# denix56/SI-Mamba

Measured on AMD Instinct MI355X. Metric: point-clouds/sec (fwd+bwd), higher is better.
Workload: dtype f32; 1 GPU; PointMamba classifier train step (FPS+kNN grouping, encoder, spectral SAST ordering, 12 Mamba blocks d=384 at L=1024, head, AdamW), 1024 pts -> 128 patches; global_batch=64, per_gpu_batch=64, npoints=1024, patches=128, mamba_seq_len=1024, parallelism=dp1, communicator_ranks=1, library_gemm=tuned solution table (si_mamba_amd/tuned/gemm_gfx950.csv)

## Files before the change

include/simamba.h:

```cpp
#ifndef SIMAMBA_H_
#define SIMAMBA_H_

#include <stddef.h>

#ifdef __cplusplus
extern "C" {
#endif

#define SIMAMBA_ABI_VERSION 9

#define SIMAMBA_F32  0
#define SIMAMBA_BF16 1

#define SIMAMBA_OK            0
#define SIMAMBA_E_NULLPTR    -1
#define SIMAMBA_E_SHAPE      -2
#define SIMAMBA_E_DTYPE      -3
#define SIMAMBA_E_DSTATE     -4
#define SIMAMBA_E_WIDTH      -5
#define SIMAMBA_E_WORKSPACE  -6
#define SIMAMBA_E_GROUPS     -7
#define SIMAMBA_E_ALIGN      -8
#define SIMAMBA_E_VARIANT    -9

#define SIMAMBA_SCAN_CHUNK 128

#define SIMAMBA_SCAN_CKPT_ROW 128
#define SIMAMBA_SCAN_CKPT_SEQ 16

int         simamba_abi_version(void);
const char* simamba_strerror(int rc);
int         simamba_scan_num_chunks(int seqlen);
int         simamba_scan_fwd_auto_variant(int batch, int dim);
int         simamba_scan_ckpt_step(int batch, int dim, int seqlen, int dstate, int io_dtype);
long long   simamba_scan_ckpt_floats(int batch, int dim, int seqlen, int dstate, int ckpt_step);

#define SIMAMBA_SCAN_AUTO    0
#define SIMAMBA_SCAN_ROWSCAN 1
#define SIMAMBA_SCAN_LPC2    2
#define SIMAMBA_SCAN_LPC4    4
#define SIMAMBA_SCAN_MIX     6
int simamba_selective_scan_fwd(const void* u, const void* delta, const float* A,
                               const void* B, const void* C, const float* D, const void* z,
                               const float* delta_bias, void* out, float* x_ckpt,
                               float* last_state, int batch, int dim, int seqlen, int dstate,
                               int io_dtype, int delta_softplus, long long z_bstride,
                               long long bc_bstride, long long bc_nstride, long long bc_tstride,
                               int ckpt_step, int variant, void* stream);

int simamba_selective_scan_bwd(const void* u, const void* delta, const float* A,
                               const void* B, const void* C, const float* D, const void* z,
                               const float* delta_bias, const void* dout, const float* x_ckpt,
                               void* du, void* ddelta, float* dA, float* dB, float* dC,
                               float* dD, void* dz, float* ddelta_bias,
                               int batch, int dim, int seqlen, int dstate,
                               int io_dtype, int delta_softplus, long long z_bstride,
                               long long dz_bstride, long long bc_bstride, long long bc_nstride,
                               long long bc_tstride, int ckpt_step, void* stream);

int simamba_selective_scan_dt_fwd(const void* u, const void* xdbl, const void* wdt, const float* A, const float* D,
                                  const void* z, const float* delta_bias, void* out, float* x_ckpt, float* last_state,
                                  int batch, int dim, int seqlen, int dstate, int dt_rank, int io_dtype,
                                  long long z_bstride, long long xdbl_bstride, long long xdbl_tstride, int ckpt_step,
                                  int variant, void* stream);
int simamba_selective_scan_dt_bwd(const void* u, const void* xdbl, const void* wdt, const float* A, const float* D,
                                  const void* z, const float* delta_bias, const void* dout, const float* x_ckpt,
                                  void* du, void* ddelta, float* dA, float* dB, float* dC, float* dD, void* dz,
                                  float* ddelta_bias, int batch, int dim, int seqlen, int dstate, int dt_rank,
                                  int io_dtype, long long z_bstride, long long dz_bstride, long long xdbl_bstride,
                                  long long xdbl_tstride, void* stream);

int simamba_xdt_proj_fwd(const void* x, const void* wx, const void* wdt, void* xdbl, void* delta,
                         int batch, int D, int seqlen, int S, int R, int io_dtype, long long x_bstride,
                         void* stream);
int simamba_conv_xdt_proj_fwd(const void* x, const float* cw, const float* cb, const void* wx, const void* wdt,
                              void* xconv, void* xdbl, void* delta, int batch, int D, int seqlen, int S, int R,
                              int io_dtype, long long x_bstride, void* stream);

int simamba_seq_gather_fwd(const void* in, const int* idx, void* out, int batch, int channels, int G, int L,
                           long long out_bstride, int io_dtype, void* stream);
int simamba_seq_gather_bwd(const void* dout, const int* inv, void* din, int batch, int channels, int G, int L,
                           int R, long long dout_bstride, int io_dtype, void* stream);

int simamba_causal_conv1d_fwd(const void* x, const float* w, const float* bias, void* out,
                              int batch, int dim, int seqlen, int width, int silu,
                              int io_dtype, long long x_bstride, void* stream);
int simamba_causal_conv1d_bwd(const void* x, const float* w, const float* bias,
                              const void* dout, void* dx, float* dw, float* dbias,
                              int batch, int dim, int seqlen, int width, int silu,
                              int io_dtype, long long x_bstride, long long dx_bstride, void* stream);

int simamba_add_layer_norm_grid(int batch, int rows_per_batch);
int simamba_add_layer_norm_fwd(const void* hidden, const float* residual, const float* rowscale,
                               const float* weight, const float* bias, float* residual_out,
                               void* normed, float* mean, float* rstd, int batch, int rows_per_batch,
                               int dim, float eps, int hidden_dtype, int out_dtype, void* stream);
int simamba_add_layer_norm_bwd(const void* dnormed, const float* dresidual_out,
                               const float* residual_out, const float* mean, const float* rstd,
                               const float* weight, const float* rowscale, float* dresidual,
                               void* dhidden, float* dwb_partial, int batch, int rows_per_batch,
                               int dim, int hidden_dtype, int out_dtype, void* stream);

int simamba_out_proj_add_ln_fwd(const void* y, const void* w, const float* residual, const float* rowscale,
                                const float* gamma, const float* beta, float* residual_out, void* normed, float* mean,
                                float* rstd, int batch, int K, int L, int C, float eps, int out_dtype, void* stream);

int simamba_in_proj_fwd(const void* x, const void* w, void* xz, int batch, int L, int C, int M, int io_dtype,
                        void* stream);

int simamba_bn_relu_grid(long long rows);
int simamba_bn_relu_fwd(const void* x, const float* gterm, int group, const float* weight, const float* bias,
                        float* running_mean, float* running_var, float momentum, float eps, int training,
                        void* y, float* mean, float* invstd, float* partial, long long rows, int C,
                        long long ld, int io_dtype, void* stream);
int simamba_bn_relu_bwd(const void* dy, const void* x, const float* gterm, int group, const float* weight,
                        const float* bias, const float* mean, const float* invstd, void* dx, float* dgterm,
                        int dgroup, float* dweight, float* dbias, float* partial, long long rows, int C,
                        long long ld, int io_dtype, int training, void* stream);
int simamba_group_max_fwd(const void* x, void* out, unsigned char* idx, long long groups, int n, int C,
                          int io_dtype, void* stream);
int simamba_group_max_bwd(const void* dout, const unsigned char* idx, void* dx, long long groups, int n, int C,
                          int io_dtype, void* stream);

int simamba_three_nn(const float* xyz1, const float* xyz2, int* idx, float* weight, int batch, int N, int S,
                     void* stream);
int simamba_three_interpolate_fwd(const void* feats, const int* idx, const float* weight, void* out, int batch,
                                  int N, int S, int C, int io_dtype, void* stream);
int simamba_three_interpolate_bwd(const void* dout, const int* idx, const float* weight, float* dfeats, int batch,
                                  int N, int S, int C, int io_dtype, void* stream);

int simamba_chamfer_fwd(const float* pred, const float* gt, float* dist, unsigned char* idx1, unsigned char* idx2,
                        long long pairs, int n, int m, void* stream);
int simamba_chamfer_bwd(const float* pred, const float* gt, const float* ddist, const unsigned char* idx1,
                        const unsigned char* idx2, float* dpred, long long pairs, int n, int m, void* stream);

int simamba_knn_group(const float* points, const float* centers, long long* idx, int batch, int N, int G, int K,
                      void* stream);

#define SIMAMBA_SPEC_SYMMETRIC   0x01u
#define SIMAMBA_SPEC_SELF_LOOP   0x02u
#define SIMAMBA_SPEC_BINARY      0x04u
#define SIMAMBA_SPEC_MATRIX_SYM  0x08u
#define SIMAMBA_SPEC_SMALLEST    0x10u
#define SIMAMBA_SPEC_SIGMA_MEAN  0x20u

int simamba_knn_graph(const float* points, float* adj, void* workspace, size_t ws_bytes,
                      int B, int G, int F, int knn, float alpha, unsigned flags, void* stream);

int simamba_laplacian_topk(const float* adj, float* evals, float* evecs, long long* order,
                           float* all_evals, float* all_evecs, int B, int G, int k,
                           unsigned flags, void* stream);

size_t simamba_spectral_workspace_bytes(int B, int G);

int simamba_spectral_topk(const float* centers, float* evals, float* evecs, long long* order,
                          void* workspace, size_t ws_bytes, int B, int G, int knn, float alpha,
                          int k, unsigned flags, void* stream);

int simamba_farthest_point_sample(const float* points, long long* idx, float* centers, int B, int N,
                                  int K, void* stream);

int simamba_argsort_rows(const float* vals, long long* idx, int rows, int n, void* stream);

#ifdef __cplusplus
}
#endif
#endif
```

si_mamba_amd/_lib.py:

```python
from __future__ import annotations

import ctypes
import os
from ctypes import c_char_p, c_float, c_int, c_longlong, c_size_t, c_uint, c_void_p

_HERE = os.path.dirname(os.path.abspath(__file__))
LIB_PATH = os.path.join(_HERE, "libsimamba_hip.so")

F32, BF16 = 0, 1

SPEC_SYMMETRIC = 0x01
SPEC_SELF_LOOP = 0x02
SPEC_BINARY = 0x04
SPEC_MATRIX_SYM = 0x08
SPEC_SMALLEST = 0x10
SPEC_SIGMA_MEAN = 0x20

SCAN_AUTO, SCAN_ROWSCAN, SCAN_LPC2, SCAN_LPC4, SCAN_MIX = 0, 1, 2, 4, 6
CKPT_ROW, CKPT_SEQ = 128, 16

_P = c_void_p
_LL = c_longlong
ABI_VERSION = 9
SIGNATURES = {
    "simamba_abi_version": (c_int, []),
    "simamba_strerror": (c_char_p, [c_int]),
    "simamba_scan_num_chunks": (c_int, [c_int]),
    "simamba_scan_fwd_auto_variant": (c_int, [c_int, c_int]),
    "simamba_scan_ckpt_step": (c_int, [c_int, c_int, c_int, c_int, c_int]),
    "simamba_scan_ckpt_floats": (_LL, [c_int, c_int, c_int, c_int, c_int]),
    "simamba_selective_scan_fwd": (c_int, [_P, _P, _P, _P, _P, _P, _P, _P, _P, _P, _P,
                                           c_int, c_int, c_int, c_int, c_int, c_int,
                                           _LL, _LL, _LL, _LL, c_int, c_int, _P]),
    "simamba_selective_scan_bwd": (c_int, [_P, _P, _P, _P, _P, _P, _P, _P, _P, _P,
                                           _P, _P, _P, _P, _P, _P, _P, _P,
                                           c_int, c_int, c_int, c_int, c_int, c_int,
                                           _LL, _LL, _LL, _LL, _LL, c_int, _P]),
    "simamba_selective_scan_dt_fwd": (c_int, [_P, _P, _P, _P, _P, _P, _P, _P, _P, _P,
                                              c_int, c_int, c_int, c_int, c_int, c_int,
                                              _LL, _LL, _LL, c_int, c_int, _P]),
    "simamba_selective_scan_dt_bwd": (c_int, [_P, _P, _P, _P, _P, _P, _P, _P, _P,
                                              _P, _P, _P, _P, _P, _P, _P, _P,
                                              c_int, c_int, c_int, c_int, c_int, c_int,
                                              _LL, _LL, _LL, _LL, _P]),
    "simamba_xdt_proj_fwd": (c_int, [_P, _P, _P, _P, _P, c_int, c_int, c_int, c_int, c_int, c_int, _LL, _P]),
    "simamba_conv_xdt_proj_fwd": (c_int, [_P, _P, _P, _P, _P, _P, _P, _P, c_int, c_int, c_int, c_int, c_int, c_int, _LL,
                                          _P]),
    "simamba_seq_gather_fwd": (c_int, [_P, _P, _P, c_int, c_int, c_int, c_int, _LL, c_int, _P]),
    "simamba_seq_gather_bwd": (c_int, [_P, _P, _P, c_int, c_int, c_int, c_int, c_int, _LL, c_int, _P]),
    "simamba_causal_conv1d_fwd": (c_int, [_P, _P, _P, _P, c_int, c_int, c_int, c_int, c_int, c_int, _LL, _P]),
    "simamba_causal_conv1d_bwd": (c_int, [_P, _P, _P, _P, _P, _P, _P,
                                          c_int, c_int, c_int, c_int, c_int, c_int, _LL, _LL, _P]),
    "simamba_add_layer_norm_grid": (c_int, [c_int, c_int]),
    "simamba_add_layer_norm_fwd": (c_int, [_P, _P, _P, _P, _P, _P, _P, _P, _P, c_int, c_int, c_int, c_float,
                                           c_int, c_int, _P]),
    "simamba_add_layer_norm_bwd": (c_int, [_P, _P, _P, _P, _P, _P, _P, _P, _P, _P, c_int, c_int, c_int,
                                           c_int, c_int, _P]),
    "simamba_out_proj_add_ln_fwd": (c_int, [_P, _P, _P, _P, _P, _P, _P, _P, _P, _P, c_int, c_int, c_int, c_int, c_float,
                                            c_int, _P]),
    "simamba_in_proj_fwd": (c_int, [_P, _P, _P, c_int, c_int, c_int, c_int, c_int, _P]),
    "simamba_bn_relu_grid": (c_int, [_LL]),
    "simamba_bn_relu_fwd": (c_int, [_P, _P, c_int, _P, _P, _P, _P, c_float, c_float, c_int, _P, _P, _P, _P, _LL, c_int,
                                    _LL, c_int, _P]),
    "simamba_bn_relu_bwd": (c_int, [_P, _P, _P, c_int, _P, _P, _P, _P, _P, _P, c_int, _P, _P, _P, _LL, c_int, _LL,
                                    c_int, c_int, _P]),
    "simamba_group_max_fwd": (c_int, [_P, _P, _P, _LL, c_int, c_int, c_int, _P]),
    "simamba_group_max_bwd": (c_int, [_P, _P, _P, _LL, c_int, c_int, c_int, _P]),
    "simamba_three_nn": (c_int, [_P, _P, _P, _P, c_int, c_int, c_int, _P]),
    "simamba_three_interpolate_fwd": (c_int, [_P, _P, _P, _P, c_int, c_int, c_int, c_int, c_int, _P]),
    "simamba_three_interpolate_bwd": (c_int, [_P, _P, _P, _P, c_int, c_int, c_int, c_int, c_int, _P]),
    "simamba_chamfer_fwd": (c_int, [_P, _P, _P, _P, _P, _LL, c_int, c_int, _P]),
    "simamba_chamfer_bwd": (c_int, [_P, _P, _P, _P, _P, _P, _LL, c_int, c_int, _P]),
    "simamba_knn_group": (c_int, [_P, _P, _P, c_int, c_int, c_int, c_int, _P]),
    "simamba_knn_graph": (c_int, [_P, _P, _P, c_size_t, c_int, c_int, c_int, c_int, c_float, c_uint, _P]),
    "simamba_laplacian_topk": (c_int, [_P, _P, _P, _P, _P, _P, c_int, c_int, c_int, c_uint, _P]),
    "simamba_spectral_workspace_bytes": (c_size_t, [c_int, c_int]),
    "simamba_spectral_topk": (c_int, [_P, _P, _P, _P, _P, c_size_t, c_int, c_int, c_int, c_float,
                                      c_int, c_uint, _P]),
    "simamba_argsort_rows": (c_int, [_P, _P, c_int, c_int, _P]),
    "simamba_farthest_point_sample": (c_int, [_P, _P, _P, c_int, c_int, c_int, _P]),
}

_lib = None


def load():
    global _lib
    if _lib is not None:
        return _lib
    if not os.path.exists(LIB_PATH):
        raise RuntimeError(
            f"{LIB_PATH} not found: build it with `python -c 'import __graft_entry__ as g; g.build()'` "
            "or `make -C si_mamba_amd/csrc`.  si_mamba_amd has no CPU / eager fallback.")
    lib = ctypes.CDLL(LIB_PATH)
    for name, (res, args) in SIGNATURES.items():
        fn = getattr(lib, name)
        fn.restype = res
        fn.argtypes = args
    got = lib.simamba_abi_version()
    if got != ABI_VERSION:
        raise RuntimeError(f"libsimamba_hip.so ABI version {got}, binding expects {ABI_VERSION}")
    _lib = lib
    return lib


def check(rc: int, what: str):
    if rc != 0:
        msg = load().simamba_strerror(rc).decode()
        raise RuntimeError(f"{what} failed (rc={rc}): {msg}")


def ptr(t):
    return None if t is None else t.data_ptr()


def dtype_code(dtype):
    import torch
    if dtype == torch.float32:
        return F32
    if dtype == torch.bfloat16:
        return BF16
    raise TypeError(f"si_mamba_amd kernels take float32 or bfloat16 activations, got {dtype}")


def stream_ptr(device):
    import torch
    return torch.cuda.current_stream(device).cuda_stream


def require_gpu(t, what):
    if not t.is_cuda:
        raise RuntimeError(
            f"{what}: tensor is on {t.device}; si_mamba_amd runs on a ROCm device only "
            "(no CPU fallback -- the CPU restatement lives in oracle/ and is test-only)")


_timing = {"on": False, "events": {}, "only": None}


def enable_kernel_timing(on=True, only=None):
    _timing["on"] = bool(on)
    _timing["events"] = {}
    _timing["only"] = None if only is None else frozenset(only)


class timed:
    __slots__ = ("name", "dev", "ev")

    def __init__(self, name, device):
        self.name, self.dev, self.ev = name, device, None

    def __enter__(self):
        if _timing["on"] and (_timing["only"] is None or self.name in _timing["only"]):
            import torch
            a, b = torch.cuda.Event(enable_timing=True), torch.cuda.Event(enable_timing=True)
            a.record(torch.cuda.current_stream(self.dev))
            self.ev = (a, b)
        return self

    def __exit__(self, *exc):
        if self.ev is not None:
            import torch
            self.ev[1].record(torch.cuda.current_stream(self.dev))
            _timing["events"].setdefault(self.name, []).append(self.ev)
        return False


def kernel_times():
    out = {}
    for name, evs in _timing["events"].items():
        ms = [a.elapsed_time(b) for a, b in evs]
        out[name] = (len(ms), sum(ms) / max(len(ms), 1))
    return out


_scan_variant = [SCAN_AUTO]


class scan_variant:

    def __init__(self, variant):
        self.v, self.prev = int(variant), None

    def __enter__(self):
        self.prev, _scan_variant[0] = _scan_variant[0], self.v
        return self

    def __exit__(self, *exc):
        _scan_variant[0] = self.prev
        return False


def current_scan_variant():
    return _scan_variant[0]


_scan_ckpt = [0]


class scan_ckpt:

    def __init__(self, step):
        self.v, self.prev = int(step), None

    def __enter__(self):
        self.prev, _scan_ckpt[0] = _scan_ckpt[0], self.v
        return self

    def __exit__(self, *exc):
        _scan_ckpt[0] = self.prev
        return False


_fuse_dt = [None]
counters = {}


def count(name):
    counters[name] = counters.get(name, 0) + 1



class scan_fuse_dt:

    def __init__(self, on):
        self.v, self.prev = (None if on is None else bool(on)), None

    def __enter__(self):
        self.prev, _fuse_dt[0] = _fuse_dt[0], self.v
        return self

    def __exit__(self, *exc):
        _fuse_dt[0] = self.prev
        return False


def fuse_dt_enabled(dtype):
    import torch
    return (dtype == torch.bfloat16) if _fuse_dt[0] is None else _fuse_dt[0]


_fuse_out_norm = [True]
_hand_in_proj = [None]


class fuse_out_norm:

    def __init__(self, on):
        self.v, self.prev = bool(on), None

    def __enter__(self):
        self.prev, _fuse_out_norm[0] = _fuse_out_norm[0], self.v
        return self

    def __exit__(self, *exc):
        _fuse_out_norm[0] = self.prev
        return False


def fuse_out_norm_enabled():
    return _fuse_out_norm[0]


class hand_in_proj:

    def __init__(self, on):
        self.v, self.prev = (None if on is None else bool(on)), None

    def __enter__(self):
        self.prev, _hand_in_proj[0] = _hand_in_proj[0], self.v
        return self

    def __exit__(self, *exc):
        _hand_in_proj[0] = self.prev
        return False


def in_proj_hand_enabled(workgroups, dtype=None):
    import torch
    if _hand_in_proj[0] is not None:
        return _hand_in_proj[0]
    return dtype != torch.float32 and workgroups >= IN_PROJ_MIN_WORKGROUPS


IN_PROJ_MIN_WORKGROUPS = 192


def scan_plan(batch, dim, seqlen, dstate, dtype, aligned, device, need_grad):
    import torch
    lib = load()
    code = dtype_code(dtype)
    step = _scan_ckpt[0] or lib.simamba_scan_ckpt_step(batch, dim, seqlen, dstate, code)
    if step == CKPT_SEQ and not (aligned and dstate == 16 and dim % 64 == 0 and
                                 seqlen % (4 if code == F32 else 8) == 0):
        step = CKPT_ROW
    if _scan_variant[0] == SCAN_ROWSCAN:
        step = CKPT_ROW
    if not need_grad:
        return step, None
    n = lib.simamba_scan_ckpt_floats(batch, dim, seqlen, dstate, step)
    return step, (torch.empty(n, device=device, dtype=torch.float32) if n else None)


def scan_bwd_accumulators(batch, dim, seqlen, dstate, has_D, has_bias, device):
    import torch
    sizes = [dim * dstate, batch * dstate * seqlen, batch * dstate * seqlen, dim if has_D else 0,
             dim if has_bias else 0]
    flat = torch.empty(sum(sizes), device=device, dtype=torch.float32)
    parts, o = [], 0
    for n in sizes:
        parts.append(flat[o:o + n])
        o += n
    dA = parts[0].view(dim, dstate)
    dB = parts[1].view(batch, dstate, seqlen)
    dC = parts[2].view(batch, dstate, seqlen)
    return dA, dB, dC, (parts[3] if has_D else None), (parts[4] if has_bias else None)
```

si_mamba_amd/mamba_inner.py:

```python
from __future__ import annotations

import torch

from . import _lib


def _w(t, dtype):
    return t if t.dtype == dtype else t.to(dtype)


def _wx(W, X):
    return torch.bmm(W.unsqueeze(0).expand(X.shape[0], -1, -1), X)


def _xw(X, W):
    return torch.bmm(X, W.unsqueeze(0).expand(X.shape[0], -1, -1))


def _sum_bmm(X, Y):
    return torch.bmm(X, Y).sum(0, dtype=torch.float32)


class InProjFn(torch.autograd.Function):

    @staticmethod
    def forward(ctx, hidden, weight, bias):
        io = hidden.dtype
        if torch.is_autocast_enabled("cuda"):
            io = torch.get_autocast_dtype("cuda")
            hidden = hidden.to(io)
        wc = _w(weight, io)
        xz = tokens_times_weight(hidden, wc) if bias is None else _wx(wc, hidden.transpose(1, 2))
        if bias is not None:
            xz = xz + _w(bias, io)[None, :, None]
        ctx.save_for_backward(hidden, weight)
        ctx.wc = wc
        ctx.has_bias = bias is not None
        return xz

    @staticmethod
    def backward(ctx, dxz):
        hidden, weight = ctx.saved_tensors
        io = hidden.dtype
        dxz = dxz.to(io)
        dh = _xw(dxz.transpose(1, 2), ctx.wc) if ctx.needs_input_grad[0] else None
        dw = _sum_bmm(dxz, hidden).to(weight.dtype) if ctx.needs_input_grad[1] else None
        db = dxz.sum((0, 2)).to(weight.dtype) if ctx.has_bias else None
        return dh, dw, db


def tokens_times_weight(x, w):
    if (x.dtype in (torch.bfloat16, torch.float32) and w.dtype == x.dtype and x.is_cuda and x.dim() == 3
            and x.is_contiguous() and in_proj_hand_ok(x, w)):
        lib = _lib.load()
        Bsz, L, C = x.shape
        wcc = w.contiguous()
        out = torch.empty(Bsz, w.shape[0], L, device=x.device, dtype=x.dtype)
        with torch.cuda.device(x.device), _lib.timed("in_proj_fwd", x.device):
            rc = lib.simamba_in_proj_fwd(x.data_ptr(), wcc.data_ptr(), out.data_ptr(), Bsz, L, C, w.shape[0],
                                         _lib.dtype_code(x.dtype), _lib.stream_ptr(x.device))
        _lib.check(rc, "simamba_in_proj_fwd")
        _lib.count("in_proj_hand")
        return out
    return _wx(w, x.transpose(1, 2))


def in_proj_hand_ok(hidden, wc):
    Bsz, L, C = hidden.shape
    tile = 128 if hidden.dtype == torch.float32 else 256
    return (C % 64 == 0 and C <= 384 and wc.shape[0] % 32 == 0 and L % 8 == 0 and hidden.data_ptr() % 16 == 0
            and _lib.in_proj_hand_enabled(Bsz * ((L + tile - 1) // tile), hidden.dtype))


def in_proj_fn(hidden, weight, bias=None):
    return InProjFn.apply(hidden, weight, bias)


def xdt_proj_fused_ok(x, wx, wdt, conv=False):
    S, D = wx.shape
    R = wdt.shape[1]
    pack = 4 if x.dtype == torch.float32 else 8
    return (x.is_cuda and x.dtype in (torch.float32, torch.bfloat16) and wx.dtype == x.dtype and wdt.dtype == x.dtype
            and x.dim() == 3 and x.stride(2) == 1 and x.stride(1) == x.shape[2] and x.stride(0) % pack == 0
            and x.shape[1] == D and D % 64 == 0 and x.shape[2] % pack == 0 and S % 4 == 0 and S <= 64
            and D * x.shape[2] * 4 < 2 ** 32 - 65536 and (not conv or D <= 1024)
            and R % 4 == 0 and 4 <= R <= 24 and S >= R and wdt.shape[0] == D and x.data_ptr() % 16 == 0)


def xdt_proj_fwd(x, wx, wdt, conv=None, want_delta=True):
    lib = _lib.load()
    Bsz, D, L = x.shape
    S, R = wx.shape[0], wdt.shape[1]
    wxc, wdc = wx.contiguous(), wdt.contiguous()
    x_dbl = torch.empty(Bsz, L, S, device=x.device, dtype=x.dtype)
    delta = torch.empty(Bsz, D, L, device=x.device, dtype=x.dtype) if want_delta else None
    with torch.cuda.device(x.device), _lib.timed("xdt_proj_fwd", x.device):
        if conv is None:
            rc = lib.simamba_xdt_proj_fwd(x.data_ptr(), wxc.data_ptr(), wdc.data_ptr(), x_dbl.data_ptr(),
                                          _lib.ptr(delta), Bsz, D, L, S, R, _lib.dtype_code(x.dtype), x.stride(0),
                                          _lib.stream_ptr(x.device))
        else:
            cw, cb, out = conv
            rc = lib.simamba_conv_xdt_proj_fwd(x.data_ptr(), cw.data_ptr(), _lib.ptr(cb), wxc.data_ptr(), wdc.data_ptr(),
                                               out.data_ptr(), x_dbl.data_ptr(), _lib.ptr(delta), Bsz, D, L, S, R,
                                               _lib.dtype_code(x.dtype), x.stride(0), _lib.stream_ptr(x.device))
    _lib.check(rc, "simamba_xdt_proj_fwd")
    return x_dbl, delta


class MambaInnerFn(torch.autograd.Function):
    @staticmethod
    def forward(ctx, xz, conv_w, conv_b, x_proj_w, dt_proj_w, out_proj_w, out_proj_b, A, D, delta_bias,
                dt_rank, d_state, grad_mode=True):
        _lib.require_gpu(xz, "mamba_inner_fn")
        lib = _lib.load()
        if xz.stride(2) != 1 or xz.stride(1) != xz.shape[2]:
            xz = xz.contiguous()
        io = xz.dtype
        code = _lib.dtype_code(io)
        Bsz, twoD, L = xz.shape
        Dm = twoD // 2
        R, N = dt_rank, d_state
        S = R + 2 * N
        dev = xz.device
        stream = _lib.stream_ptr(dev)
        xbs = xz.stride(0)
        x_in, z = xz[:, :Dm], xz[:, Dm:]

        cw = conv_w.float().contiguous()
        cb = None if conv_b is None else conv_b.float().contiguous()
        Af = A.float().contiguous()
        Df = None if D is None else D.float().contiguous()
        bf = None if delta_bias is None else delta_bias.float().contiguous()
        W = cw.shape[1]

        no_out = out_proj_w is None
        xw_c, dtw_c = _w(x_proj_w, io), _w(dt_proj_w, io)
        ow_c = None if no_out else _w(out_proj_w, io)
        ctx.wcast = (xw_c, dtw_c, ow_c)
        x_conv = torch.empty(Bsz, Dm, L, device=dev, dtype=io)
        need_grad = grad_mode and any(ctx.needs_input_grad)
        pack = 4 if io == torch.float32 else 8
        aligned = xz.data_ptr() % 16 == 0 and (xbs * xz.element_size()) % 16 == 0
        ckpt_step, x_ckpt = _lib.scan_plan(Bsz, Dm, L, N, io, aligned, dev, need_grad)
        fuse_dt = (_lib.fuse_dt_enabled(io) and ckpt_step == _lib.CKPT_SEQ and N == 16 and R % pack == 0 and R <= 24
                   and _lib.current_scan_variant() != _lib.SCAN_ROWSCAN)
        if W == 4 and xdt_proj_fused_ok(x_in, xw_c, dtw_c, conv=True):
            x_dbl, delta = xdt_proj_fwd(x_in, xw_c, dtw_c, conv=(cw, cb, x_conv), want_delta=not fuse_dt)
        else:
            fuse_dt = False
            with torch.cuda.device(dev), _lib.timed("conv1d_fwd", dev):
                rc = lib.simamba_causal_conv1d_fwd(x_in.data_ptr(), cw.data_ptr(), _lib.ptr(cb), x_conv.data_ptr(),
                                                   Bsz, Dm, L, W, 1, code, xbs, stream)
            _lib.check(rc, "simamba_causal_conv1d_fwd")
            if xdt_proj_fused_ok(x_conv, xw_c, dtw_c):
                x_dbl, delta = xdt_proj_fwd(x_conv, xw_c, dtw_c)
            else:
                x_dbl = _xw(x_conv.transpose(1, 2), xw_c.t())
                delta = _wx(dtw_c, x_dbl[:, :, :R].transpose(1, 2))
        Bv, Cv = x_dbl[:, :, R:R + N], x_dbl[:, :, R + N:]
        if x_dbl.data_ptr() % 16:
            raise RuntimeError("mamba_inner_fn: unaligned x_proj output")

        y = torch.empty(Bsz, Dm, L, device=dev, dtype=io)
        dtw_k = dtw_c.contiguous() if fuse_dt else None
        with torch.cuda.device(dev), _lib.timed("scan_fwd", dev):
            if fuse_dt:
                _lib.count("scan_dt_fwd")
                rc = lib.simamba_selective_scan_dt_fwd(
                    x_conv.data_ptr(), x_dbl.data_ptr(), dtw_k.data_ptr(), Af.data_ptr(), _lib.ptr(Df),
                    z.data_ptr(), _lib.ptr(bf), y.data_ptr(), _lib.ptr(x_ckpt), None,
                    Bsz, Dm, L, N, R, code, xbs, x_dbl.stride(0), x_dbl.stride(1),
                    ckpt_step, _lib.current_scan_variant(), stream)
            else:
                rc = lib.simamba_selective_scan_fwd(
                    x_conv.data_ptr(), delta.data_ptr(), Af.data_ptr(), Bv.data_ptr(), Cv.data_ptr(), _lib.ptr(Df),
                    z.data_ptr(), _lib.ptr(bf), y.data_ptr(), _lib.ptr(x_ckpt), None,
                    Bsz, Dm, L, N, code, 1, xbs, x_dbl.stride(0), 1, x_dbl.stride(1),
                    ckpt_step, _lib.current_scan_variant(), stream)
        _lib.check(rc, "simamba_selective_scan_fwd")

        if no_out:
            out = y
        else:
            out = _xw(y.transpose(1, 2), ow_c.t())
            if out_proj_b is not None:
                out = out + _w(out_proj_b, io)
        ctx.no_out = no_out
        ctx.dims = (R, N, W)
        ctx.ckpt_step = ckpt_step
        ctx.dtw_k = dtw_k
        ctx.has_out_bias = out_proj_b is not None and not no_out
        ctx.param_dtypes = (conv_w.dtype, None if conv_b is None else conv_b.dtype, x_proj_w.dtype,
                            dt_proj_w.dtype, None if no_out else out_proj_w.dtype, A.dtype,
                            None if D is None else D.dtype, None if delta_bias is None else delta_bias.dtype)
        ctx.save_for_backward(xz, x_conv, x_dbl, delta, None if no_out else y, cw, cb, x_proj_w, dt_proj_w, out_proj_w,
                              Af, Df, bf, x_ckpt)
        return out

    @staticmethod
    def backward(ctx, dout):
        (xz, x_conv, x_dbl, delta, y, cw, cb, x_proj_w, dt_proj_w, out_proj_w, Af, Df, bf, x_ckpt) = ctx.saved_tensors
        lib = _lib.load()
        R, N, W = ctx.dims
        io = xz.dtype
        code = _lib.dtype_code(io)
        Bsz, twoD, L = xz.shape
        Dm = twoD // 2
        S = R + 2 * N
        dev = xz.device
        stream = _lib.stream_ptr(dev)
        xbs = xz.stride(0)
        dout = dout.to(io)
        f32 = dict(device=dev, dtype=torch.float32)
        xw_c, dtw_c, ow_c = ctx.wcast
        if ctx.no_out:
            dy = dout.contiguous()
            d_out_w = d_out_b = None
        else:
            if dout.stride(2) != 1:
                dout = dout.contiguous()
            d_out_w = _sum_bmm(dout.transpose(1, 2), y.transpose(1, 2))
            d_out_b = dout.sum((0, 1)) if ctx.has_out_bias else None
            dy = tokens_times_weight(dout, ow_c.t())

        dxz = torch.empty_like(xz)
        du = torch.empty(Bsz, Dm, L, device=dev, dtype=io)
        ddelta = torch.empty(Bsz, Dm, L, device=dev, dtype=io)
        dA, dB, dC, dD, dbias = _lib.scan_bwd_accumulators(Bsz, Dm, L, N, Df is not None, bf is not None, dev)
        Bv, Cv = x_dbl[:, :, R:R + N], x_dbl[:, :, R + N:]
        z, dz = xz[:, Dm:], dxz[:, Dm:]
        with torch.cuda.device(dev), _lib.timed("scan_bwd", dev):
            if ctx.dtw_k is not None:
                rc = lib.simamba_selective_scan_dt_bwd(
                    x_conv.data_ptr(), x_dbl.data_ptr(), ctx.dtw_k.data_ptr(), Af.data_ptr(), _lib.ptr(Df),
                    z.data_ptr(), _lib.ptr(bf), dy.data_ptr(), _lib.ptr(x_ckpt),
                    du.data_ptr(), ddelta.data_ptr(), dA.data_ptr(), dB.data_ptr(), dC.data_ptr(), _lib.ptr(dD),
                    dz.data_ptr(), _lib.ptr(dbias), Bsz, Dm, L, N, R, code,
                    xbs, dxz.stride(0), x_dbl.stride(0), x_dbl.stride(1), stream)
            else:
                rc = lib.simamba_selective_scan_bwd(
                    x_conv.data_ptr(), delta.data_ptr(), Af.data_ptr(), Bv.data_ptr(), Cv.data_ptr(), _lib.ptr(Df),
                    z.data_ptr(), _lib.ptr(bf), dy.data_ptr(), _lib.ptr(x_ckpt),
                    du.data_ptr(), ddelta.data_ptr(), dA.data_ptr(), dB.data_ptr(), dC.data_ptr(), _lib.ptr(dD),
                    dz.data_ptr(), _lib.ptr(dbias), Bsz, Dm, L, N, code, 1,
                    xbs, dxz.stride(0), x_dbl.stride(0), 1, x_dbl.stride(1), ctx.ckpt_step, stream)
        _lib.check(rc, "simamba_selective_scan_bwd")

        dx_dbl = torch.empty(Bsz, L, S, device=dev, dtype=io)
        dx_dbl[:, :, :R].copy_(_xw(ddelta.transpose(1, 2), dtw_c))
        dBC = torch.as_strided(dB, (2, Bsz, N, L), (Bsz * N * L, N * L, L, 1))
        dx_dbl[:, :, R:].view(Bsz, L, 2, N).copy_(dBC.permute(1, 3, 0, 2))
        d_dt_w = _sum_bmm(ddelta, x_dbl[:, :, :R])
        d_x_w = _sum_bmm(dx_dbl.transpose(1, 2), x_conv.transpose(1, 2))
        wxT = xw_c.t().unsqueeze(0).expand(Bsz, -1, -1)
        torch.baddbmm(du, wxT, dx_dbl.transpose(1, 2), out=du)

        dconv = torch.empty(Dm * W + (Dm if cb is not None else 0), **f32)
        dcw = dconv[:Dm * W].view(Dm, W)
        dcb = dconv[Dm * W:] if cb is not None else None
        with torch.cuda.device(dev), _lib.timed("conv1d_bwd", dev):
            rc = lib.simamba_causal_conv1d_bwd(xz.data_ptr(), cw.data_ptr(), _lib.ptr(cb), du.data_ptr(),
                                               dxz.data_ptr(), dcw.data_ptr(), _lib.ptr(dcb),
                                               Bsz, Dm, L, W, 1, code, xbs, dxz.stride(0), stream)
        _lib.check(rc, "simamba_causal_conv1d_bwd")

        t_cw, t_cb, t_xw, t_dtw, t_ow, t_A, t_D, t_b = ctx.param_dtypes
        return (dxz, dcw.to(t_cw), None if dcb is None else dcb.to(t_cb), d_x_w.to(t_xw), d_dt_w.to(t_dtw),
                None if d_out_w is None else d_out_w.to(t_ow),
                None if d_out_b is None else d_out_b.to(out_proj_w.dtype), dA.to(t_A),
                None if dD is None else dD.to(t_D), None if dbias is None else dbias.to(t_b), None, None, None)


def mamba_inner_fn(xz, conv1d_weight, conv1d_bias, x_proj_weight, delta_proj_weight, out_proj_weight,
                   out_proj_bias, A, D=None, delta_bias=None, dt_rank=None, d_state=None):
    if conv1d_weight.dim() == 3:
        conv1d_weight = conv1d_weight.squeeze(1)
    if dt_rank is None:
        dt_rank = delta_proj_weight.shape[1]
    if d_state is None:
        d_state = (x_proj_weight.shape[0] - dt_rank) // 2
    return MambaInnerFn.apply(xz, conv1d_weight, conv1d_bias, x_proj_weight, delta_proj_weight, out_proj_weight,
                              out_proj_bias, A, D, delta_bias, dt_rank, d_state, torch.is_grad_enabled())
```

Baseline: 1123 point-clouds/s.

## Add bf16x3 split-precision MFMA GEMM for f32 in/out projections

Adds HIP kernels that split f32 weights into three bf16 planes and run the f32 in_proj and out_proj GEMMs (forward and the backward input-gradient) on bf16 MFMA using six products per tile, emulating f32 accuracy. Activations are split on the fly inside the kernel while staging into LDS, with double buffering. The path turns on when batch*L reaches 32768 tokens, which the default workload meets (64*1024). It aims to replace slower f32 library or hand GEMMs with matrix-core throughput, at the cost of extra splitting work each step and slightly different rounding from true f32.

```diff
diff --git a/include/simamba.h b/include/simamba.h
--- a/include/simamba.h
+++ b/include/simamba.h
@@ -108,6 +108,11 @@
 int simamba_in_proj_fwd(const void* x, const void* w, void* xz, int batch, int L, int C, int M, int io_dtype,
                         void* stream);
 
+int simamba_split_bf16x3(const float* w, int rows, int cols, long long row_stride, long long col_stride, void* planes,
+                         void* planes_t, void* stream);
+int simamba_gemm_split_tok(const void* x, const void* wplanes, void* out, int batch, int L, int K, int M, void* stream);
+int simamba_gemm_split_chan(const void* x, const void* wplanes, void* out, int batch, int L, int K, int N, void* stream);
+
 int simamba_bn_relu_grid(long long rows);
 int simamba_bn_relu_fwd(const void* x, const float* gterm, int group, const float* weight, const float* bias,
                         float* running_mean, float* running_var, float momentum, float eps, int training,
diff --git a/si_mamba_amd/_lib.py b/si_mamba_amd/_lib.py
--- a/si_mamba_amd/_lib.py
+++ b/si_mamba_amd/_lib.py
@@ -59,6 +59,9 @@
     "simamba_out_proj_add_ln_fwd": (c_int, [_P, _P, _P, _P, _P, _P, _P, _P, _P, _P, c_int, c_int, c_int, c_int, c_float,
                                             c_int, _P]),
     "simamba_in_proj_fwd": (c_int, [_P, _P, _P, c_int, c_int, c_int, c_int, c_int, _P]),
+    "simamba_split_bf16x3": (c_int, [_P, c_int, c_int, _LL, _LL, _P, _P, _P]),
+    "simamba_gemm_split_tok": (c_int, [_P, _P, _P, c_int, c_int, c_int, c_int, _P]),
+    "simamba_gemm_split_chan": (c_int, [_P, _P, _P, c_int, c_int, c_int, c_int, _P]),
     "simamba_bn_relu_grid": (c_int, [_LL]),
     "simamba_bn_relu_fwd": (c_int, [_P, _P, c_int, _P, _P, _P, _P, c_float, c_float, c_int, _P, _P, _P, _P, _LL, c_int,
                                     _LL, c_int, _P]),
@@ -276,6 +279,10 @@
         return False
 
 
+def hand_in_proj_forced():
+    return _hand_in_proj[0]
+
+
 def in_proj_hand_enabled(workgroups, dtype=None):
     import torch
     if _hand_in_proj[0] is not None:
@@ -284,6 +291,32 @@
 
 
 IN_PROJ_MIN_WORKGROUPS = 192
+
+
+_split_gemm = [None]
+
+
+class split_gemm:
+
+    def __init__(self, on):
+        self.v, self.prev = (None if on is None else bool(on)), None
+
+    def __enter__(self):
+        self.prev, _split_gemm[0] = _split_gemm[0], self.v
+        return self
+
+    def __exit__(self, *exc):
+        _split_gemm[0] = self.prev
+        return False
+
+
+def split_gemm_enabled(tokens):
+    if _split_gemm[0] is not None:
+        return _split_gemm[0]
+    return tokens >= SPLIT_GEMM_MIN_TOKENS
+
+
+SPLIT_GEMM_MIN_TOKENS = 32768
 
 
 def scan_plan(batch, dim, seqlen, dstate, dtype, aligned, device, need_grad):
diff --git a/si_mamba_amd/csrc/split_gemm.hip b/si_mamba_amd/csrc/split_gemm.hip
--- /dev/null
+++ b/si_mamba_amd/csrc/split_gemm.hip
@@ -0,0 +1,281 @@
+#include "common.h"
+
+namespace simamba {
+
+typedef float sg_f32x16 __attribute__((ext_vector_type(16)));
+typedef __bf16 sg_bf16x8 __attribute__((ext_vector_type(8)));
+typedef __bf16 sg_bf16x2 __attribute__((ext_vector_type(2)));
+typedef float sg_f32x2 __attribute__((ext_vector_type(2)));
+
+constexpr int kSgThreads = 256;
+constexpr int kSgT = 128;
+constexpr int kSgKS = 16;
+constexpr int kSgPitch = kSgKS + 8;
+constexpr int kSgPlane = kSgT * kSgPitch;
+
+__device__ __forceinline__ unsigned sg_pk(float a, float b) {
+  return __builtin_bit_cast(unsigned, __builtin_convertvector((sg_f32x2){a, b}, sg_bf16x2));
+}
+__device__ __forceinline__ void sg_split2(float a, float b, unsigned& h, unsigned& m, unsigned& l) {
+  h = sg_pk(a, b);
+  a -= __uint_as_float(h << 16);
+  b -= __uint_as_float(h & 0xffff0000u);
+  m = sg_pk(a, b);
+  a -= __uint_as_float(m << 16);
+  b -= __uint_as_float(m & 0xffff0000u);
+  l = sg_pk(a, b);
+}
+
+struct SgArgs {
+  const float* x;
+  const uint16_t* w;
+  float* out;
+  int batch, L, K, nch;
+};
+
+template <bool kA>
+__global__ __launch_bounds__(kSgThreads, 2) void split_gemm_kernel(SgArgs p) {
+  __shared__ __attribute__((aligned(16))) uint16_t sX[2][3][kSgPlane];
+  __shared__ __attribute__((aligned(16))) uint16_t sW[2][3][kSgPlane];
+  const int tid = threadIdx.x;
+  const int lane = tid & 63;
+  const int wave = __builtin_amdgcn_readfirstlane(tid >> 6);
+  const int li = lane & 31, hh = lane >> 5;
+  const int L = p.L, K = p.K, nch = p.nch;
+
+  const unsigned n = gridDim.x;
+  unsigned bid = blockIdx.x;
+  if (n % 8 == 0) bid = (bid % 8) * (n / 8) + bid / 8;
+  const int nct = (nch + kSgT - 1) / kSgT;
+  const int tps = (L + kSgT - 1) / kSgT;
+  const int ct = static_cast<int>(bid % static_cast<unsigned>(nct));
+  const int rest = static_cast<int>(bid / static_cast<unsigned>(nct));
+  const int b = rest / tps;
+  const int t0 = (rest - b * tps) * kSgT;
+  const int c0 = ct * kSgT;
+
+  const float* xb = p.x + static_cast<size_t>(b) * L * K;
+  const size_t wplane = static_cast<size_t>(nch) * K;
+
+  const int wr = tid >> 1, wc = 8 * (tid & 1);
+  const uint16_t* wsrc = p.w + static_cast<size_t>(c0 + wr < nch ? c0 + wr : nch - 1) * K + wc;
+  const int wdst = wr * kSgPitch + wc;
+
+  const float* xsrc[2];
+  int xdst[2];
+  if constexpr (kA) {
+#pragma unroll
+    for (int i = 0; i < 2; ++i) {
+      const int q = tid + kSgThreads * i;
+      const int r = q >> 2, t = t0 + r;
+      xsrc[i] = xb + static_cast<size_t>(t < L ? t : L - 1) * K + 4 * (q & 3);
+      xdst[i] = r * kSgPitch + 4 * (q & 3);
+    }
+  } else {
+    const int kp = tid & 7, tc = 4 * (tid >> 3);
+    const int t = t0 + tc < L ? t0 + tc : L - 4;
+#pragma unroll
+    for (int i = 0; i < 2; ++i) xsrc[i] = xb + static_cast<size_t>(2 * kp + i) * L + t;
+    xdst[0] = tc * kSgPitch + 2 * kp;
+    xdst[1] = 0;
+  }
+
+  struct Stage { float4 x[2]; uint4 w[3]; };
+  auto load = [&](Stage& s, int ks) __attribute__((always_inline)) {
+    const int k0 = ks * kSgKS;
+#pragma unroll
+    for (int pl = 0; pl < 3; ++pl) s.w[pl] = *reinterpret_cast<const uint4*>(wsrc + pl * wplane + k0);
+    if constexpr (kA) {
+#pragma unroll
+      for (int i = 0; i < 2; ++i) s.x[i] = *reinterpret_cast<const float4*>(xsrc[i] + k0);
+    } else {
+#pragma unroll
+      for (int i = 0; i < 2; ++i) s.x[i] = *reinterpret_cast<const float4*>(xsrc[i] + static_cast<size_t>(k0) * L);
+    }
+  };
+  auto store = [&](const Stage& s, int buf) __attribute__((always_inline)) {
+#pragma unroll
+    for (int pl = 0; pl < 3; ++pl) *reinterpret_cast<uint4*>(&sW[buf][pl][wdst]) = s.w[pl];
+    if constexpr (kA) {
+#pragma unroll
+      for (int i = 0; i < 2; ++i) {
+        unsigned h0, m0, l0, h1, m1, l1;
+        sg_split2(s.x[i].x, s.x[i].y, h0, m0, l0);
+        sg_split2(s.x[i].z, s.x[i].w, h1, m1, l1);
+        *reinterpret_cast<uint2*>(&sX[buf][0][xdst[i]]) = make_uint2(h0, h1);
+        *reinterpret_cast<uint2*>(&sX[buf][1][xdst[i]]) = make_uint2(m0, m1);
+        *reinterpret_cast<uint2*>(&sX[buf][2][xdst[i]]) = make_uint2(l0, l1);
+      }
+    } else {
+      const float* r0 = reinterpret_cast<const float*>(&s.x[0]);
+      const float* r1 = reinterpret_cast<const float*>(&s.x[1]);
+#pragma unroll
+      for (int e = 0; e < 4; ++e) {
+        unsigned h, m, l;
+        sg_split2(r0[e], r1[e], h, m, l);
+        const int d = xdst[0] + e * kSgPitch;
+        *reinterpret_cast<unsigned*>(&sX[buf][0][d]) = h;
+        *reinterpret_cast<unsigned*>(&sX[buf][1][d]) = m;
+        *reinterpret_cast<unsigned*>(&sX[buf][2][d]) = l;
+      }
+    }
+  };
+
+  const int wi = wave & 1, wj = wave >> 1;
+  const int ioff = (64 * wi + li) * kSgPitch + 8 * hh;
+  const int joff = (64 * wj + li) * kSgPitch + 8 * hh;
+
+  sg_f32x16 accH[2][2], accS[2][2];
+#pragma unroll
+  for (int r = 0; r < 2; ++r)
+#pragma unroll
+    for (int c = 0; c < 2; ++c)
+#pragma unroll
+      for (int e = 0; e < 16; ++e) accH[r][c][e] = accS[r][c][e] = 0.f;
+
+  auto compute = [&](int buf, auto&& mid) __attribute__((always_inline)) {
+    const uint16_t* sI = kA ? &sX[buf][0][0] : &sW[buf][0][0];
+    const uint16_t* sJ = kA ? &sW[buf][0][0] : &sX[buf][0][0];
+    sg_bf16x8 fa[3][2], fb[3][2];
+#pragma unroll
+    for (int pl = 0; pl < 3; ++pl)
+#pragma unroll
+      for (int r = 0; r < 2; ++r) {
+        fa[pl][r] = *reinterpret_cast<const sg_bf16x8*>(sI + pl * kSgPlane + ioff + 32 * r * kSgPitch);
+        fb[pl][r] = *reinterpret_cast<const sg_bf16x8*>(sJ + pl * kSgPlane + joff + 32 * r * kSgPitch);
+      }
+#ifndef SG_STORE_AFTER
+    mid();
+#endif
+#pragma unroll
+    for (int r = 0; r < 2; ++r) {
+#pragma unroll
+      for (int c = 0; c < 2; ++c) {
+        sg_f32x16 s = accS[r][c];
+        s = __builtin_amdgcn_mfma_f32_32x32x16_bf16(fa[2][r], fb[0][c], s, 0, 0, 0);
+        s = __builtin_amdgcn_mfma_f32_32x32x16_bf16(fa[0][r], fb[2][c], s, 0, 0, 0);
+        s = __builtin_amdgcn_mfma_f32_32x32x16_bf16(fa[1][r], fb[1][c], s, 0, 0, 0);
+        s = __builtin_amdgcn_mfma_f32_32x32x16_bf16(fa[1][r], fb[0][c], s, 0, 0, 0);
+        s = __builtin_amdgcn_mfma_f32_32x32x16_bf16(fa[0][r], fb[1][c], s, 0, 0, 0);
+        accS[r][c] = s;
+        accH[r][c] = __builtin_amdgcn_mfma_f32_32x32x16_bf16(fa[0][r], fb[0][c], accH[r][c], 0, 0, 0);
+      }
+    }
+#ifdef SG_STORE_AFTER
+    mid();
+#endif
+  };
+
+  const int nks = K / kSgKS;
+  Stage sa, sb;
+  load(sa, 0);
+  load(sb, nks > 1 ? 1 : 0);
+  store(sa, 0);
+  load(sa, nks > 2 ? 2 : nks - 1);
+  __syncthreads();
+  for (int ks = 0; ks < nks; ks += 2) {
+    compute(0, [&] { if (ks + 1 < nks) store(sb, 1); });
+    load(sb, ks + 3 < nks ? ks + 3 : nks - 1);
+    __syncthreads();
+    if (ks + 1 < nks) {
+      compute(1, [&] { if (ks + 2 < nks) store(sa, 0); });
+      load(sa, ks + 4 < nks ? ks + 4 : nks - 1);
+      __syncthreads();
+    }
+  }
+
+#pragma unroll
+  for (int r = 0; r < 2; ++r)
+#pragma unroll
+    for (int c = 0; c < 2; ++c) {
+      const int jj = 64 * wj + 32 * c + li;
+#pragma unroll
+      for (int g = 0; g < 4; ++g) {
+        const int ii = 64 * wi + 32 * r + 8 * g + 4 * hh;
+        float4 v;
+        v.x = accH[r][c][4 * g + 0] + accS[r][c][4 * g + 0];
+        v.y = accH[r][c][4 * g + 1] + accS[r][c][4 * g + 1];
+        v.z = accH[r][c][4 * g + 2] + accS[r][c][4 * g + 2];
+        v.w = accH[r][c][4 * g + 3] + accS[r][c][4 * g + 3];
+        if constexpr (kA) {
+          const int t = t0 + ii, ch = c0 + jj;
+          if (t < L && ch < nch)
+            *reinterpret_cast<float4*>(p.out + (static_cast<size_t>(b) * nch + ch) * L + t) = v;
+        } else {
+          const int t = t0 + jj, ch = c0 + ii;
+          if (t < L && ch < nch)
+            *reinterpret_cast<float4*>(p.out + (static_cast<size_t>(b) * L + t) * nch + ch) = v;
+        }
+      }
+    }
+}
+
+__global__ __launch_bounds__(256) void split_bf16x3_kernel(const float* __restrict__ w, int rows, int cols, long long rs,
+                                                           long long cs, uint16_t* __restrict__ planes,
+                                                           uint16_t* __restrict__ planes_t) {
+  const long long n = static_cast<long long>(rows) * cols;
+  const long long i = static_cast<long long>(blockIdx.x) * blockDim.x + threadIdx.x;
+  const bool tr = blockIdx.y == 1;
+  uint16_t* const dst = tr ? planes_t : planes;
+  if (i >= n || !dst) return;
+  const int inner = tr ? rows : cols;
+  const int o = static_cast<int>(i / inner), q = static_cast<int>(i - static_cast<long long>(o) * inner);
+  const int r = tr ? q : o, c = tr ? o : q;
+  unsigned h, m, l;
+  sg_split2(w[r * rs + c * cs], 0.f, h, m, l);
+  dst[i] = static_cast<uint16_t>(h);
+  dst[n + i] = static_cast<uint16_t>(m);
+  dst[2 * n + i] = static_cast<uint16_t>(l);
+}
+
+static int sg_check(const void* x, const void* w, const void* out, int batch, int L, int K, int nch) {
+  if (batch < 0 || L < 0 || K <= 0 || nch <= 0) return SIMAMBA_E_SHAPE;
+  if (K % kSgKS || nch % 32 || L % 4) return SIMAMBA_E_SHAPE;
+  if (static_cast<long long>(K) * L >= (1LL << 29) || static_cast<long long>(nch) * L >= (1LL << 29) ||
+      static_cast<long long>(nch) * K >= (1LL << 29))
+    return SIMAMBA_E_SHAPE;
+  const long long tiles =
+      static_cast<long long>(batch) * ((L + kSgT - 1) / kSgT) * ((nch + kSgT - 1) / kSgT);
+  if (tiles > 0x7fffffffLL) return SIMAMBA_E_SHAPE;
+  if (batch == 0 || L == 0) return SIMAMBA_OK;
+  if (!x || !w || !out) return SIMAMBA_E_NULLPTR;
+  if ((reinterpret_cast<uintptr_t>(x) | reinterpret_cast<uintptr_t>(w) | reinterpret_cast<uintptr_t>(out)) & 15u)
+    return SIMAMBA_E_ALIGN;
+  return 1;
+}
+
+template <bool kA>
+static int sg_launch(const void* x, const void* w, void* out, int batch, int L, int K, int nch, void* stream) {
+  const int rc = sg_check(x, w, out, batch, L, K, nch);
+  if (rc != 1) return rc;
+  SgArgs a{static_cast<const float*>(x), static_cast<const uint16_t*>(w), static_cast<float*>(out), batch, L, K, nch};
+  const unsigned tiles =
+      static_cast<unsigned>(batch) * ((L + kSgT - 1) / kSgT) * ((nch + kSgT - 1) / kSgT);
+  hipLaunchKernelGGL((split_gemm_kernel<kA>), dim3(tiles), dim3(kSgThreads), 0, static_cast<hipStream_t>(stream), a);
+  return static_cast<int>(hipGetLastError());
+}
+
+}
+
+using namespace simamba;
+
+extern "C" int simamba_split_bf16x3(const float* w, int rows, int cols, long long row_stride, long long col_stride,
+                                    void* planes, void* planes_t, void* stream) {
+  if (rows <= 0 || cols <= 0 || static_cast<long long>(rows) * cols >= (1LL << 29)) return SIMAMBA_E_SHAPE;
+  if (!w || (!planes && !planes_t)) return SIMAMBA_E_NULLPTR;
+  const long long n = static_cast<long long>(rows) * cols;
+  hipLaunchKernelGGL(split_bf16x3_kernel, dim3(static_cast<unsigned>((n + 255) / 256), 2), dim3(256), 0,
+                     static_cast<hipStream_t>(stream), w, rows, cols, row_stride, col_stride,
+                     static_cast<uint16_t*>(planes), static_cast<uint16_t*>(planes_t));
+  return static_cast<int>(hipGetLastError());
+}
+
+extern "C" int simamba_gemm_split_tok(const void* x, const void* wplanes, void* out, int batch, int L, int K, int M,
+                                      void* stream) {
+  return sg_launch<true>(x, wplanes, out, batch, L, K, M, stream);
+}
+
+extern "C" int simamba_gemm_split_chan(const void* x, const void* wplanes, void* out, int batch, int L, int K, int N,
+                                       void* stream) {
+  return sg_launch<false>(x, wplanes, out, batch, L, K, N, stream);
+}
diff --git a/si_mamba_amd/mamba_inner.py b/si_mamba_amd/mamba_inner.py
--- a/si_mamba_amd/mamba_inner.py
+++ b/si_mamba_amd/mamba_inner.py
@@ -30,7 +30,12 @@
             io = torch.get_autocast_dtype("cuda")
             hidden = hidden.to(io)
         wc = _w(weight, io)
-        xz = tokens_times_weight(hidden, wc) if bias is None else _wx(wc, hidden.transpose(1, 2))
+        ctx.wplanes_t = None
+        if bias is None and split_tok_ok(hidden, wc.shape[0]):
+            planes, ctx.wplanes_t = split_weight(wc, both=ctx.needs_input_grad[0])
+            xz = split_tok(hidden, planes)
+        else:
+            xz = tokens_times_weight(hidden, wc) if bias is None else _wx(wc, hidden.transpose(1, 2))
         if bias is not None:
             xz = xz + _w(bias, io)[None, :, None]
         ctx.save_for_backward(hidden, weight)
@@ -43,13 +48,20 @@
         hidden, weight = ctx.saved_tensors
         io = hidden.dtype
         dxz = dxz.to(io)
-        dh = _xw(dxz.transpose(1, 2), ctx.wc) if ctx.needs_input_grad[0] else None
+        dh = None
+        if ctx.needs_input_grad[0]:
+            if split_chan_ok(dxz, ctx.wc.shape[1]):
+                dh = split_chan(dxz, ctx.wplanes_t if ctx.wplanes_t is not None else split_weight(ctx.wc.t())[0])
+            else:
+                dh = _xw(dxz.transpose(1, 2), ctx.wc)
         dw = _sum_bmm(dxz, hidden).to(weight.dtype) if ctx.needs_input_grad[1] else None
         db = dxz.sum((0, 2)).to(weight.dtype) if ctx.has_bias else None
         return dh, dw, db
 
 
-def tokens_times_weight(x, w):
+def tokens_times_weight(x, w, planes=None):
+    if split_tok_ok(x, w.shape[0]):
+        return split_tok(x, planes if planes is not None else split_weight(w)[0])
     if (x.dtype in (torch.bfloat16, torch.float32) and w.dtype == x.dtype and x.is_cuda and x.dim() == 3
             and x.is_contiguous() and in_proj_hand_ok(x, w)):
         lib = _lib.load()
@@ -70,6 +82,58 @@
     tile = 128 if hidden.dtype == torch.float32 else 256
     return (C % 64 == 0 and C <= 384 and wc.shape[0] % 32 == 0 and L % 8 == 0 and hidden.data_ptr() % 16 == 0
             and _lib.in_proj_hand_enabled(Bsz * ((L + tile - 1) // tile), hidden.dtype))
+
+
+def split_weight(w, both=False):
+    lib = _lib.load()
+    R, C = w.shape
+    planes = torch.empty(3, R, C, device=w.device, dtype=torch.bfloat16)
+    planes_t = torch.empty(3, C, R, device=w.device, dtype=torch.bfloat16) if both else None
+    with torch.cuda.device(w.device):
+        rc = lib.simamba_split_bf16x3(w.data_ptr(), R, C, w.stride(0), w.stride(1), planes.data_ptr(),
+                                      _lib.ptr(planes_t), _lib.stream_ptr(w.device))
+    _lib.check(rc, "simamba_split_bf16x3")
+    return planes, planes_t
+
+
+def _split_ok(x, L, K, nch):
+    return (x.dtype == torch.float32 and x.is_cuda and x.dim() == 3 and x.is_contiguous() and x.data_ptr() % 16 == 0
+            and K % 16 == 0 and nch % 32 == 0 and L % 4 == 0 and K * L < 2 ** 29 and nch * L < 2 ** 29
+            and nch * K < 2 ** 29 and _lib.split_gemm_enabled(x.shape[0] * L))
+
+
+def split_tok_ok(x, nch):
+    return _lib.hand_in_proj_forced() is None and _split_ok(x, x.shape[1], x.shape[2], nch)
+
+
+def split_chan_ok(x, nch):
+    return _split_ok(x, x.shape[2], x.shape[1], nch)
+
+
+def split_tok(x, planes):
+    lib = _lib.load()
+    Bsz, L, K = x.shape
+    M = planes.shape[1]
+    out = torch.empty(Bsz, M, L, device=x.device, dtype=torch.float32)
+    with torch.cuda.device(x.device), _lib.timed("split_gemm_tok", x.device):
+        rc = lib.simamba_gemm_split_tok(x.data_ptr(), planes.data_ptr(), out.data_ptr(), Bsz, L, K, M,
+                                        _lib.stream_ptr(x.device))
+    _lib.check(rc, "simamba_gemm_split_tok")
+    _lib.count("split_gemm_tok")
+    return out
+
+
+def split_chan(x, planes):
+    lib = _lib.load()
+    Bsz, K, L = x.shape
+    N = planes.shape[1]
+    out = torch.empty(Bsz, L, N, device=x.device, dtype=torch.float32)
+    with torch.cuda.device(x.device), _lib.timed("split_gemm_chan", x.device):
+        rc = lib.simamba_gemm_split_chan(x.data_ptr(), planes.data_ptr(), out.data_ptr(), Bsz, L, K, N,
+                                         _lib.stream_ptr(x.device))
+    _lib.check(rc, "simamba_gemm_split_chan")
+    _lib.count("split_gemm_chan")
+    return out
 
 
 def in_proj_fn(hidden, weight, bias=None):
@@ -135,6 +199,7 @@
         W = cw.shape[1]
 
         no_out = out_proj_w is None
+        ctx.ow_planes_t = None
         xw_c, dtw_c = _w(x_proj_w, io), _w(dt_proj_w, io)
         ow_c = None if no_out else _w(out_proj_w, io)
         ctx.wcast = (xw_c, dtw_c, ow_c)
@@ -183,7 +248,11 @@
         if no_out:
             out = y
         else:
-            out = _xw(y.transpose(1, 2), ow_c.t())
+            if split_chan_ok(y, ow_c.shape[0]):
+                planes, ctx.ow_planes_t = split_weight(ow_c, both=need_grad)
+                out = split_chan(y, planes)
+            else:
+                out = _xw(y.transpose(1, 2), ow_c.t())
             if out_proj_b is not None:
                 out = out + _w(out_proj_b, io)
         ctx.no_out = no_out
@@ -222,7 +291,7 @@
                 dout = dout.contiguous()
             d_out_w = _sum_bmm(dout.transpose(1, 2), y.transpose(1, 2))
             d_out_b = dout.sum((0, 1)) if ctx.has_out_bias else None
-            dy = tokens_times_weight(dout, ow_c.t())
+            dy = tokens_times_weight(dout, ow_c.t(), ctx.ow_planes_t)
 
         dxz = torch.empty_like(xz)
         du = torch.empty(Bsz, Dm, L, device=dev, dtype=io)
```

Result: faster. 1144 point-clouds/s (median of 6 runs) (+1.9%).
